# tenpy/cyten

Hardware: AMD Instinct MI355X
Metric: block-sparse tdot+SVD GFLOP/s (fp64) (higher is better)
Workload: dtype f64

## Files before the change

cyten_amd/csrc/blocked_qr.hip:

```cpp
#include "blocked_qr.h"
#include "qr_strip_chunks.h"

#include <algorithm>
#include <cstdlib>
#include <utility>

namespace cyb {
namespace {

#define GLOBAL_AS __attribute__((address_space(1)))
typedef GLOBAL_AS double* gp;
typedef const GLOBAL_AS double* gcp;
typedef double d4 __attribute__((ext_vector_type(4)));

constexpr int PNT = 512;
constexpr int PNW = PNT / 64;

__device__ __forceinline__ double wave_sum(double v)
{
#pragma unroll
    for (int o = 32; o > 0; o >>= 1) v += __shfl_xor(v, o);
    return v;
}

struct PanelDesc {
    double* Ac;
    double* V;
    double* T;
    double* tau;
    int64_t ld;
    int32_t m, j0, pw, pad;
    double* ctl = nullptr;
    const double* parts = nullptr;
    double rel2 = 0.0;
    int32_t n_parts = 0, step = 0;
};
constexpr int PANEL_V_ZEROED = 1;
constexpr int PANEL_REFLECT_ALWAYS = 2;

__global__ void __launch_bounds__(PNT) qr_panel_kernel(const PanelDesc* __restrict__ descs)
{
    __shared__ double red[PNW];
    __shared__ double s_tau, s_scale;
    __shared__ double Ts[NBK][NBK + 1];
    __shared__ double z[NBK];
    __shared__ double taus[NBK];
    const PanelDesc d = descs[blockIdx.x];
    const int tid = threadIdx.x, lane = tid & 63, wave = tid >> 6;
    gp Ac = (gp)d.Ac;
    gp V = (gp)d.V;
    const int64_t ld = d.ld;
    const int m = d.m, j0 = d.j0, pw = d.pw;
    for (int e = tid; e < NBK * (NBK + 1); e += PNT) (&Ts[0][0])[e] = 0.0;

    for (int jj = 0; jj < pw; ++jj) {
        const int col = j0 + jj;
        gp x = Ac + (int64_t)col * ld + col;
        const int L = m - col;
        double mx = 0.0;
        for (int i = 1 + tid; i < L; i += PNT) mx = fmax(mx, fabs(x[i]));
#pragma unroll
        for (int o = 32; o > 0; o >>= 1) mx = fmax(mx, __shfl_xor(mx, o));
        if (lane == 0) red[wave] = mx;
        __syncthreads();
        mx = 0.0;
#pragma unroll
        for (int q = 0; q < PNW; ++q) mx = fmax(mx, red[q]);
        __syncthreads();
        double ss = 0.0;
        if (mx > 1e-290) {
            const double inv = 1.0 / mx;
            for (int i = 1 + tid; i < L; i += PNT) {
                const double t = x[i] * inv;
                ss += t * t;
            }
        }
        ss = wave_sum(ss);
        if (lane == 0) red[wave] = ss;
        __syncthreads();
        if (tid == 0) {
            double tot = 0.0;
            for (int q = 0; q < PNW; ++q) tot += red[q];
            const double xnorm = mx * sqrt(tot);
            const double alpha = x[0];
            double t = 0.0, scale = 0.0, beta = alpha;
            if (xnorm != 0.0) {
                beta = -copysign(hypot(alpha, xnorm), alpha);
                t = (beta - alpha) / beta;
                scale = 1.0 / (alpha - beta);
            } else if ((d.pad & PANEL_REFLECT_ALWAYS) && alpha != 0.0) {
                beta = -alpha;
                t = 2.0;
            }
            s_tau = t;
            s_scale = scale;
            taus[jj] = t;
            ((gp)d.tau)[col] = t;
            x[0] = beta;
        }
        __syncthreads();
        const double tj = s_tau, scale = s_scale;
        gp v = V + (int64_t)col * ld;
        for (int i = tid; i < m; i += PNT) {
            double val = 0.0;
            if (i == col) val = 1.0;
            else if (i > col) val = (tj != 0.0) ? x[i - col] * scale : 0.0;
            v[i] = val;
        }
        __syncthreads();
        if (tj != 0.0) {
            for (int c = col + 1 + wave; c < j0 + pw; c += PNW) {
                gp a = Ac + (int64_t)c * ld + col;
                gcp vv = v + col;
                double dot = 0.0;
                for (int i = lane; i < L; i += 64) dot += vv[i] * a[i];
                dot = wave_sum(dot) * tj;
                for (int i = lane; i < L; i += 64) a[i] -= dot * vv[i];
            }
        }
        for (int i = wave; i < jj; i += PNW) {
            gcp vi = V + (int64_t)(j0 + i) * ld;
            double dot = 0.0;
            for (int r = col + lane; r < m; r += 64) dot += vi[r] * v[r];
            dot = wave_sum(dot);
            if (lane == 0) z[i] = dot;
        }
        __syncthreads();
        if (tid < jj) {
            double acc = 0.0;
            for (int l = tid; l < jj; ++l) acc += Ts[tid][l] * z[l];
            Ts[tid][jj] = -tj * acc;
        }
        if (tid == 0) Ts[jj][jj] = tj;
        __syncthreads();
    }
    for (int e = tid; e < NBK * NBK; e += PNT) ((gp)d.T)[e] = Ts[e / NBK][e % NBK];
}

#ifndef CYB_QR_READLANE
#define CYB_QR_READLANE 1
#endif
constexpr int RP_NT = 512;
constexpr int RP_RPT = 3;
constexpr int RP_NW = RP_NT / 64;

__device__ __forceinline__ double dshfl_xor(double v, int m) { return __shfl_xor(v, m); }

#ifndef CYB_QR_REDUCE_DPP
#define CYB_QR_REDUCE_DPP 1
#endif
#if CYB_QR_REDUCE_DPP
__device__ __forceinline__ void dswap32(double& a, double& b)
{
    const auto lo = __builtin_amdgcn_permlane32_swap((unsigned)__double2loint(a), (unsigned)__double2loint(b), false, false);
    const auto hi = __builtin_amdgcn_permlane32_swap((unsigned)__double2hiint(a), (unsigned)__double2hiint(b), false, false);
    a = __hiloint2double((int)hi[0], (int)lo[0]);
    b = __hiloint2double((int)hi[1], (int)lo[1]);
}
__device__ __forceinline__ void dswap16(double& a, double& b)
{
    const auto lo = __builtin_amdgcn_permlane16_swap((unsigned)__double2loint(a), (unsigned)__double2loint(b), false, false);
    const auto hi = __builtin_amdgcn_permlane16_swap((unsigned)__double2hiint(a), (unsigned)__double2hiint(b), false, false);
    a = __hiloint2double((int)hi[0], (int)lo[0]);
    b = __hiloint2double((int)hi[1], (int)lo[1]);
}
template <int CTRL, int BANKS>
__device__ __forceinline__ double ddpp(double old, double src)
{
    const int lo = __builtin_amdgcn_update_dpp(__double2loint(old), __double2loint(src), CTRL, 0xf, BANKS, false);
    const int hi = __builtin_amdgcn_update_dpp(__double2hiint(old), __double2hiint(src), CTRL, 0xf, BANKS, false);
    return __hiloint2double(hi, lo);
}
__device__ __forceinline__ double reduce_scatter16(double (&v)[16], int )
{
    double a[8];
#pragma unroll
    for (int i = 0; i < 8; ++i) {
        double x = v[i], y = v[i + 8];
        dswap32(x, y);
        a[i] = x + y;
    }
    double b[4];
#pragma unroll
    for (int i = 0; i < 4; ++i) {
        double x = a[i], y = a[i + 4];
        dswap16(x, y);
        b[i] = x + y;
    }
    constexpr int ROW_MIRROR = 0x140, ROW_HALF_MIRROR = 0x141;
    double c[2];
#pragma unroll
    for (int i = 0; i < 2; ++i) {
        const double p = ddpp<ROW_MIRROR, 0xc>(b[i], b[i + 2]);
        const double q = ddpp<ROW_MIRROR, 0x3>(b[i + 2], b[i]);
        c[i] = p + q;
    }
    const double p = ddpp<ROW_HALF_MIRROR, 0xa>(c[0], c[1]);
    const double q = ddpp<ROW_HALF_MIRROR, 0x5>(c[1], c[0]);
    double d = p + q;
    d += ddpp<0x4e, 0xf>(d, d);
    d += ddpp<0xb1, 0xf>(d, d);
    return d;
}
#else
__device__ __forceinline__ double reduce_scatter16(double (&v)[16], int lane)
{
    double a[8];
    {
        const bool hi = (lane & 32) != 0;
#pragma unroll
        for (int i = 0; i < 8; ++i) {
            const double send = hi ? v[i] : v[i + 8];
            const double keep = hi ? v[i + 8] : v[i];
            a[i] = keep + dshfl_xor(send, 32);
        }
    }
    double b[4];
    {
        const bool hi = (lane & 16) != 0;
#pragma unroll
        for (int i = 0; i < 4; ++i) {
            const double send = hi ? a[i] : a[i + 4];
            const double keep = hi ? a[i + 4] : a[i];
            b[i] = keep + dshfl_xor(send, 16);
        }
    }
    double c[2];
    {
        const bool hi = (lane & 8) != 0;
#pragma unroll
        for (int i = 0; i < 2; ++i) {
            const double send = hi ? b[i] : b[i + 2];
            const double keep = hi ? b[i + 2] : b[i];
            c[i] = keep + dshfl_xor(send, 8);
        }
    }
    double d;
    {
        const bool hi = (lane & 4) != 0;
        const double send = hi ? c[0] : c[1];
        const double keep = hi ? c[1] : c[0];
        d = keep + dshfl_xor(send, 4);
    }
    d += dshfl_xor(d, 2);
    d += dshfl_xor(d, 1);
    return d;
}
#endif

struct PanelShared {
    double wred[2][RP_NW][NBK];
    double wsum[2][NBK];
    double rowb[2][NBK];
    double Zs[NBK][NBK + 1];
    double taus[NBK];
    double Ts[NBK][NBK + 1];
};

template <int JJ, int RPT, int NT>
__device__ __forceinline__ void panel_step(double (&P)[RPT][NBK], PanelShared& sh, const PanelDesc& d, int tid)
{
    if (JJ >= d.pw) return;
    const int lane = tid & 63, wave = tid >> 6;
    const int j0 = d.j0;
    const int prow = j0 + JJ;
    constexpr int pb = JJ & 1;
#pragma unroll
    for (int h = 0; h < 2; ++h) {
        double part[16];
#pragma unroll
        for (int c = 0; c < 16; ++c) part[c] = 0.0;
#pragma unroll
        for (int q = 0; q < RPT; ++q) {
            const double x = (q == 0 && tid <= JJ) ? 0.0 : P[q][JJ];
#pragma unroll
            for (int c = 0; c < 16; ++c) part[c] += x * P[q][h * 16 + c];
        }
        const double r = reduce_scatter16(part, lane);
        if ((lane & 3) == 0) {
            const int idx = ((lane >> 5) & 1) * 8 + ((lane >> 4) & 1) * 4 + ((lane >> 3) & 1) * 2 + ((lane >> 2) & 1);
            sh.wred[pb][wave][h * 16 + idx] = r;
        }
    }
    if (tid == JJ) {
#pragma unroll
        for (int c = 0; c < NBK; ++c) sh.rowb[pb][c] = P[0][c];
    }
    __syncthreads();
#if CYB_QR_READLANE
    const int lc = lane & (NBK - 1);
    double ws = 0.0;
#pragma unroll
    for (int w = 0; w < NT / 64; ++w) ws += sh.wred[pb][w][lc];
    const double rb = sh.rowb[pb][lc];
    const double alpha = __hiloint2double(__builtin_amdgcn_readlane(__double2hiint(rb), JJ), __builtin_amdgcn_readlane(__double2loint(rb), JJ));
    const double xn2_raw = __hiloint2double(__builtin_amdgcn_readlane(__double2hiint(ws), JJ), __builtin_amdgcn_readlane(__double2loint(ws), JJ));
#else
    if (tid < NBK) {
        double t = 0.0;
#pragma unroll
        for (int w = 0; w < NT / 64; ++w) t += sh.wred[pb][w][tid];
        sh.wsum[pb][tid] = t;
    }
    __syncthreads();
    const double alpha = sh.rowb[pb][JJ];
    const double xn2_raw = sh.wsum[pb][JJ];
#endif
    const double xn2 = fma(alpha * alpha, (d.pad & PANEL_REFLECT_ALWAYS) ? 1e-40 : 0.0, xn2_raw);
    double tau = 0.0, scale = 0.0, beta = alpha;
    if (xn2 > 1e-290) {
        beta = -copysign(sqrt(alpha * alpha + xn2), alpha);
        tau = (beta - alpha) / beta;
        scale = 1.0 / (alpha - beta);
    }
    double v[RPT];
#pragma unroll
    for (int q = 0; q < RPT; ++q) {
        const double x = P[q][JJ];
        if (q == 0) {
            const bool below = tid > JJ;
            const bool pivot = tid == JJ;
            v[q] = below ? x * scale : (pivot ? 1.0 : 0.0);
            P[q][JJ] = below ? v[q] : (pivot ? beta : x);
        } else {
            v[q] = x * scale;
            P[q][JJ] = v[q];
        }
    }
#if CYB_QR_READLANE
    const double tl = tau * (rb + scale * ws);
    const int tlo = __double2loint(tl), thi = __double2hiint(tl);
#pragma unroll
    for (int c = JJ + 1; c < NBK; ++c) {
        const double t = __hiloint2double(__builtin_amdgcn_readlane(thi, c), __builtin_amdgcn_readlane(tlo, c));
#pragma unroll
        for (int q = 0; q < RPT; ++q) P[q][c] -= t * v[q];
    }
#else
#pragma unroll
    for (int c = JJ + 1; c < NBK; ++c) {
        if (c < d.pw) {
            const double t = tau * (sh.rowb[pb][c] + scale * sh.wsum[pb][c]);
#pragma unroll
            for (int q = 0; q < RPT; ++q) P[q][c] -= t * v[q];
        }
    }
#endif
#if CYB_QR_READLANE
    if (tid < JJ) sh.Zs[tid][JJ] = rb + scale * ws;
#else
    if (tid < JJ) sh.Zs[tid][JJ] = sh.rowb[pb][tid] + scale * sh.wsum[pb][tid];
#endif
    if (tid == 0) {
        sh.taus[JJ] = tau;
        ((gp)d.tau)[prow] = tau;
    }
}

template <int RPT, int NT, int... Is>
__device__ __forceinline__ void panel_steps(double (&P)[RPT][NBK], PanelShared& sh, const PanelDesc& d, int tid,
                                            std::integer_sequence<int, Is...>)
{
    (panel_step<Is, RPT, NT>(P, sh, d, tid), ...);
}

template <int RPT, int NT = RP_NT>
__device__ __forceinline__ void panel_reg_body(const PanelDesc& d, PanelShared& sh, const int tid)
{
    gp Ac = (gp)d.Ac;
    gp V = (gp)d.V;
    const int64_t ld = d.ld;
    const int m = d.m, j0 = d.j0, pw = d.pw;
    double P[RPT][NBK];
#pragma unroll
    for (int q = 0; q < RPT; ++q) {
        const int row = j0 + tid + NT * q;
        const bool ok = row < m;
        gcp src = (gcp)Ac + (int64_t)j0 * ld + (ok ? row : j0);
#pragma unroll
        for (int c = 0; c < NBK; ++c) P[q][c] = src[(int64_t)(c < pw ? c : pw - 1) * ld];
#pragma unroll
        for (int c = 0; c < NBK; ++c) {
            asm volatile("" : "+v"(P[q][c]));
            P[q][c] = (ok && c < pw) ? P[q][c] : 0.0;
        }
    }
    for (int e = tid; e < NBK * (NBK + 1); e += NT) (&sh.Zs[0][0])[e] = 0.0;
    __syncthreads();

    panel_steps<RPT, NT>(P, sh, d, tid, std::make_integer_sequence<int, NBK>{});
#pragma unroll
    for (int q = 0; q < RPT; ++q) {
        const int row = j0 + tid + NT * q;
        if (row < m) {
            gp pa = Ac + (int64_t)j0 * ld + row;
            gp pv = V + (int64_t)j0 * ld + row;
#pragma unroll
            for (int c = 0; c < NBK; ++c)
                if (c < pw) {
                    pa[(int64_t)c * ld] = P[q][c];
                    pv[(int64_t)c * ld] = (q > 0 || tid > c) ? P[q][c] : (tid == c ? 1.0 : 0.0);
                }
        }
    }
    for (int64_t e = tid; e < ((d.pad & PANEL_V_ZEROED) ? 0 : (int64_t)j0 * pw); e += NT) {
        const int c = (int)(e / j0), row = (int)(e % j0);
        V[(int64_t)(j0 + c) * ld + row] = 0.0;
    }
    __syncthreads();
    if (tid < NBK) {
        double trow[NBK];
#pragma unroll
        for (int j = 0; j < NBK; ++j) {
            double acc = 0.0;
#pragma unroll
            for (int l = 0; l < j; ++l) acc += trow[l] * sh.Zs[l][j];
            const double tj = j < pw ? sh.taus[j] : 0.0;
            trow[j] = (tid < j) ? -tj * acc : (tid == j ? tj : 0.0);
            sh.Ts[tid][j] = trow[j];
        }
    }
    __syncthreads();

    for (int e = tid; e < NBK * NBK; e += NT) ((gp)d.T)[e] = sh.Ts[e / NBK][e % NBK];
}

template <int NT, typename Desc>
__device__ __forceinline__ bool panel_stop_check(const Desc& d, double* red, int tid, bool writer = true)
{
    if (!d.ctl) return false;
    gp ctl = (gp)d.ctl;
    const double stopped = ctl[0];
    if (stopped != 0.0) return (double)d.step >= stopped - 1.0;
    if (d.n_parts <= 0) return false;
    gcp parts = (gcp)d.parts;
    double t = 0.0;
    for (int i = tid; i < d.n_parts; i += NT) t += parts[i];
#pragma unroll
    for (int o = 32; o > 0; o >>= 1) t += __shfl_xor(t, o);
    if ((tid & 63) == 0) red[tid >> 6] = t;
    __syncthreads();
    double sum = 0.0;
#pragma unroll
    for (int w = 0; w < NT / 64; ++w) sum += red[w];
    const double ref = fmax(ctl[1], sum);
    const bool stop = sum <= d.rel2 * ref;
    __syncthreads();
    if (tid == 0 && writer) {
        if (stop) ctl[0] = (double)d.step + 1.0;
        else ctl[1] = ref;
    }
    return stop;
}

__global__ void __launch_bounds__(RP_NT) qr_panel_reg_kernel(const PanelDesc* __restrict__ descs)
{
    __shared__ PanelShared sh;
    const PanelDesc d = descs[blockIdx.x];
    if (panel_stop_check<RP_NT>(d, &sh.wsum[0][0], (int)threadIdx.x)) return;
    panel_reg_body<RP_RPT>(d, sh, (int)threadIdx.x);
}
struct PanelDescM {
    double* Ac;
    double* V;
    double* T;
    double* tau;
    double* xchg;
    unsigned int* ticket;
    unsigned int* err;
    int64_t ld;
    int32_t m, j0, pw, vzero;
    int32_t wg, n_wg, pad0, pad1;
    double* ctl = nullptr;
    const double* parts = nullptr;
    double rel2 = 0.0;
    int32_t n_parts = 0, step = 0;
};
constexpr int RPM_ROWS = RP_NT * RP_RPT;

template <int JJ>
__device__ __forceinline__ void panel_step_multi(double (&P)[RP_RPT][NBK], PanelShared& sh, const PanelDescM& d, int tid)
{
    if (JJ >= d.pw) return;
    const int lane = tid & 63, wave = tid >> 6;
    const int j0 = d.j0, rbase = d.j0 + d.wg * RPM_ROWS;
    const int prow = j0 + JJ;
    constexpr int pb = JJ & 1;
#pragma unroll
    for (int h = 0; h < 2; ++h) {
        double part[16];
#pragma unroll
        for (int c = 0; c < 16; ++c) part[c] = 0.0;
#pragma unroll
        for (int q = 0; q < RP_RPT; ++q) {
            const int row = rbase + tid + RP_NT * q;
            const double x = (row <= prow) ? 0.0 : P[q][JJ];
#pragma unroll
            for (int c = 0; c < 16; ++c) part[c] += x * P[q][h * 16 + c];
        }
        const double r = reduce_scatter16(part, lane);
        if ((lane & 3) == 0) {
            const int idx = ((lane >> 5) & 1) * 8 + ((lane >> 4) & 1) * 4 + ((lane >> 3) & 1) * 2 + ((lane >> 2) & 1);
            sh.wred[pb][wave][h * 16 + idx] = r;
        }
    }
#pragma unroll
    for (int q = 0; q < RP_RPT; ++q)
        if (rbase + tid + RP_NT * q == prow) {
#pragma unroll
            for (int c = 0; c < NBK; ++c) sh.rowb[pb][c] = P[q][c];
        }
    __syncthreads();
    if (tid < NBK) {
        double t = 0.0;
#pragma unroll
        for (int w = 0; w < RP_NW; ++w) t += sh.wred[pb][w][tid];
        double* slot = d.xchg + ((size_t)JJ * d.n_wg + d.wg) * 64;
        __hip_atomic_store(slot + tid, t, __ATOMIC_RELAXED, __HIP_MEMORY_SCOPE_AGENT);
        if (d.wg == 0) __hip_atomic_store(slot + 32 + tid, sh.rowb[pb][tid], __ATOMIC_RELAXED, __HIP_MEMORY_SCOPE_AGENT);
        asm volatile("s_waitcnt vmcnt(0)" ::: "memory");
        if (tid == 0) {
            __hip_atomic_fetch_add(d.ticket + JJ, 1u, __ATOMIC_RELAXED, __HIP_MEMORY_SCOPE_AGENT);
            const unsigned long long t0 = wall_clock64();
            while (__hip_atomic_load(d.ticket + JJ, __ATOMIC_RELAXED, __HIP_MEMORY_SCOPE_AGENT) < (unsigned int)d.n_wg) {
                if (wall_clock64() - t0 > 100000000ull || __hip_atomic_load(d.err, __ATOMIC_RELAXED, __HIP_MEMORY_SCOPE_AGENT)) {
                    __hip_atomic_store(d.err, 1u, __ATOMIC_RELAXED, __HIP_MEMORY_SCOPE_AGENT);
                    break;
                }
            }
        }
        asm volatile("" ::: "memory");
        __builtin_amdgcn_wave_barrier();
        double tot = 0.0;
        for (int w = 0; w < d.n_wg; ++w)
            tot += __hip_atomic_load(d.xchg + ((size_t)JJ * d.n_wg + w) * 64 + tid, __ATOMIC_RELAXED, __HIP_MEMORY_SCOPE_AGENT);
        sh.wsum[pb][tid] = tot;
        sh.rowb[pb][tid] = __hip_atomic_load(d.xchg + (size_t)JJ * d.n_wg * 64 + 32 + tid, __ATOMIC_RELAXED, __HIP_MEMORY_SCOPE_AGENT);
    }
    __syncthreads();
    const double alpha = sh.rowb[pb][JJ];
    const double xn2 = fma(alpha * alpha, (d.vzero & PANEL_REFLECT_ALWAYS) ? 1e-40 : 0.0, sh.wsum[pb][JJ]);
    double tau = 0.0, scale = 0.0, beta = alpha;
    if (xn2 > 1e-290) {
        beta = -copysign(sqrt(alpha * alpha + xn2), alpha);
        tau = (beta - alpha) / beta;
        scale = 1.0 / (alpha - beta);
    }
    double v[RP_RPT];
#pragma unroll
    for (int q = 0; q < RP_RPT; ++q) {
        const int row = rbase + tid + RP_NT * q;
        const double x = P[q][JJ];
        const bool below = row > prow;
        const bool pivot = row == prow;
        v[q] = below ? x * scale : (pivot ? 1.0 : 0.0);
        P[q][JJ] = below ? v[q] : (pivot ? beta : x);
    }
#pragma unroll
    for (int c = JJ + 1; c < NBK; ++c) {
        if (c < d.pw) {
            const double t = tau * (sh.rowb[pb][c] + scale * sh.wsum[pb][c]);
#pragma unroll
            for (int q = 0; q < RP_RPT; ++q) P[q][c] -= t * v[q];
        }
    }
    if (tid < JJ) sh.Zs[tid][JJ] = sh.rowb[pb][tid] + scale * sh.wsum[pb][tid];
    if (tid == 0) {
        sh.taus[JJ] = tau;
        if (d.wg == 0) ((gp)d.tau)[prow] = tau;
    }
}

template <int... Is>
__device__ __forceinline__ void panel_steps_multi(double (&P)[RP_RPT][NBK], PanelShared& sh, const PanelDescM& d, int tid,
                                                  std::integer_sequence<int, Is...>)
{
    (panel_step_multi<Is>(P, sh, d, tid), ...);
}

__global__ void __launch_bounds__(RP_NT) qr_panel_multi_kernel(const PanelDescM* __restrict__ descs)
{
    __shared__ PanelShared sh;
    const PanelDescM d = descs[blockIdx.x];
    const int tid = threadIdx.x;
    if (panel_stop_check<RP_NT>(d, &sh.wsum[0][0], tid, d.wg == 0)) return;
    gp Ac = (gp)d.Ac;
    gp V = (gp)d.V;
    const int64_t ld = d.ld;
    const int m = d.m, j0 = d.j0, pw = d.pw, rbase = d.j0 + d.wg * RPM_ROWS;
    double P[RP_RPT][NBK];
#pragma unroll
    for (int q = 0; q < RP_RPT; ++q) {
        const int row = rbase + tid + RP_NT * q;
#pragma unroll
        for (int c = 0; c < NBK; ++c) P[q][c] = (row < m && c < pw) ? Ac[(int64_t)(j0 + c) * ld + row] : 0.0;
    }
    for (int e = tid; e < NBK * (NBK + 1); e += RP_NT) (&sh.Zs[0][0])[e] = 0.0;
    __syncthreads();
    panel_steps_multi(P, sh, d, tid, std::make_integer_sequence<int, NBK>{});
#pragma unroll
    for (int q = 0; q < RP_RPT; ++q) {
        const int row = rbase + tid + RP_NT * q;
        if (row < m) {
#pragma unroll
            for (int c = 0; c < NBK; ++c)
                if (c < pw) {
                    const int col = j0 + c;
                    Ac[(int64_t)col * ld + row] = P[q][c];
                    V[(int64_t)col * ld + row] = (row > col) ? P[q][c] : (row == col ? 1.0 : 0.0);
                }
        }
    }
    if (d.wg == 0 && !(d.vzero & PANEL_V_ZEROED))
        for (int64_t e = tid; e < (int64_t)j0 * pw; e += RP_NT) {
            const int c = (int)(e / j0), row = (int)(e % j0);
            V[(int64_t)(j0 + c) * ld + row] = 0.0;
        }
    __syncthreads();
    if (tid < NBK) {
        double trow[NBK];
#pragma unroll
        for (int j = 0; j < NBK; ++j) {
            double acc = 0.0;
#pragma unroll
            for (int l = 0; l < j; ++l) acc += trow[l] * sh.Zs[l][j];
            const double tj = j < pw ? sh.taus[j] : 0.0;
            trow[j] = (tid < j) ? -tj * acc : (tid == j ? tj : 0.0);
            sh.Ts[tid][j] = trow[j];
        }
    }
    __syncthreads();
    if (d.wg == 0)
        for (int e = tid; e < NBK * NBK; e += RP_NT) ((gp)d.T)[e] = sh.Ts[e / NBK][e % NBK];
}

constexpr int RP_WAVE_RPT = 3;
constexpr int RP_WAVE_ROWS = 64 * RP_WAVE_RPT;
__global__ void __launch_bounds__(64) qr_panel_wave_kernel(const PanelDesc* __restrict__ descs)
{
    __shared__ PanelShared sh;
    const PanelDesc d = descs[blockIdx.x];
    if (panel_stop_check<64>(d, &sh.wsum[0][0], (int)threadIdx.x)) return;
    panel_reg_body<RP_WAVE_RPT, 64>(d, sh, (int)threadIdx.x);
}
__global__ void __launch_bounds__(128) qr_panel_wave2_kernel(const PanelDesc* __restrict__ descs)
{
    __shared__ PanelShared sh;
    const PanelDesc d = descs[blockIdx.x];
    if (panel_stop_check<128>(d, &sh.wsum[0][0], (int)threadIdx.x)) return;
    panel_reg_body<RP_WAVE_RPT, 128>(d, sh, (int)threadIdx.x);
}
__global__ void __launch_bounds__(256) qr_panel_wave4_kernel(const PanelDesc* __restrict__ descs)
{
    __shared__ PanelShared sh;
    const PanelDesc d = descs[blockIdx.x];
    if (panel_stop_check<256>(d, &sh.wsum[0][0], (int)threadIdx.x)) return;
    panel_reg_body<RP_WAVE_RPT, 256>(d, sh, (int)threadIdx.x);
}

struct StripDesc {
    double* C;
    const double* V;
    const double* T;
    int64_t ldc, ldv;
    int32_t mr, nc, pw, transT;
    const double* ctl = nullptr;
    double* part_out = nullptr;
    int32_t step = 0, pad2 = 0;
};
constexpr int ST_NT = 512;
constexpr int ST_NW = ST_NT / 64;
constexpr int ST_LS = NBK + 1;
constexpr int ST_UN = 4;

template <bool NORM>
__global__ void __launch_bounds__(ST_NT) reflector_strip_kernel(const StripDesc* __restrict__ descs)
{
    __shared__ double part[ST_NW][NBK][ST_LS];
    __shared__ double W1s[NBK][ST_LS], W2s[NBK][ST_LS], Ps[NBK][ST_LS];
    const StripDesc d = descs[blockIdx.x];
    if (d.ctl) {
        const double stopped = *(gcp)d.ctl;
        if (stopped != 0.0 && (double)d.step >= stopped - 1.0) return;
    }
    const int tid = threadIdx.x, lane = tid & 63, wave = tid >> 6;
    const int x = lane & 15, kq = lane >> 4;
    gcp V = (gcp)d.V;
    gp C = (gp)d.C;
    gcp T = (gcp)d.T;
    const int mr = d.mr, nc = d.nc, pw = d.pw;
    const int64_t ldv = d.ldv, ldc = d.ldc;
    for (int e = tid; e < NBK * NBK; e += ST_NT) {
        const int a = e / NBK, b = e % NBK;
        Ps[a][b] = T[d.transT ? b * NBK + a : e];
    }
    {
        const int64_t vo0 = (int64_t)(x < pw ? x : 0) * ldv, vo1 = (int64_t)(x + 16 < pw ? x + 16 : 0) * ldv;
        const int64_t co0 = (int64_t)(x < nc ? x : 0) * ldc, co1 = (int64_t)(x + 16 < nc ? x + 16 : 0) * ldc;
        d4 acc[2][2];
#pragma unroll
        for (int i = 0; i < 2; ++i)
#pragma unroll
            for (int j = 0; j < 2; ++j) acc[i][j] = d4{0.0, 0.0, 0.0, 0.0};
        const int nstep = (mr + 7) / 8;
        double va[ST_UN][2][2], ca[ST_UN][2][2], vn[ST_UN][2][2], cn[ST_UN][2][2];
        auto load = [&](double (&v)[ST_UN][2][2], double (&c)[ST_UN][2][2], int s0) {
#pragma unroll
            for (int u = 0; u < ST_UN; ++u) {
                const int i = (s0 + ST_NW * u) * 8 + 2 * kq;
#pragma unroll
                for (int h = 0; h < 2; ++h) {
                    const bool ok = i + h < mr;
                    const int ii = ok ? i + h : 0;
                    v[u][0][h] = ok ? V[vo0 + ii] : 0.0;
                    v[u][1][h] = ok ? V[vo1 + ii] : 0.0;
                    c[u][0][h] = ok ? C[co0 + ii] : 0.0;
                    c[u][1][h] = ok ? C[co1 + ii] : 0.0;
                }
            }
        };
        if (wave < nstep) load(va, ca, wave);
        for (int s0 = wave; s0 < nstep; s0 += ST_NW * ST_UN) {
            const bool more = s0 + ST_NW * ST_UN < nstep;
            if (more) load(vn, cn, s0 + ST_NW * ST_UN);
#pragma unroll
            for (int u = 0; u < ST_UN; ++u) {
                if (s0 + ST_NW * u < nstep) {
#pragma unroll
                    for (int h = 0; h < 2; ++h)
#pragma unroll
                        for (int i = 0; i < 2; ++i)
#pragma unroll
                            for (int j = 0; j < 2; ++j)
                                acc[i][j] = __builtin_amdgcn_mfma_f64_16x16x4f64(va[u][i][h], ca[u][j][h], acc[i][j], 0, 0, 0);
                }
            }
            if (more) {
#pragma unroll
                for (int u = 0; u < ST_UN; ++u)
#pragma unroll
                    for (int i = 0; i < 2; ++i)
#pragma unroll
                        for (int h = 0; h < 2; ++h) {
                            va[u][i][h] = vn[u][i][h];
                            ca[u][i][h] = cn[u][i][h];
                        }
            }
        }
#pragma unroll
        for (int i = 0; i < 2; ++i)
#pragma unroll
            for (int j = 0; j < 2; ++j)
#pragma unroll
                for (int r = 0; r < 4; ++r) part[wave][i * 16 + kq + 4 * r][j * 16 + x] = acc[i][j][r];
    }
    __syncthreads();
    for (int e = tid; e < NBK * NBK; e += ST_NT) {
        const int a = e / NBK, c = e % NBK;
        double t = 0.0;
#pragma unroll
        for (int w = 0; w < ST_NW; ++w) t += part[w][a][c];
        W1s[a][c] = t;
    }
    __syncthreads();
    if (wave < 4) {
        const int ta = wave >> 1, tc = wave & 1;
        d4 acc = d4{0.0, 0.0, 0.0, 0.0};
#pragma unroll
        for (int kk = 0; kk < NBK / 4; ++kk)
            acc = __builtin_amdgcn_mfma_f64_16x16x4f64(Ps[ta * 16 + x][4 * kk + kq], W1s[4 * kk + kq][tc * 16 + x], acc, 0, 0, 0);
#pragma unroll
        for (int r = 0; r < 4; ++r) W2s[ta * 16 + kq + 4 * r][tc * 16 + x] = acc[r];
    }
    __syncthreads();
    {
        double w2[2][NBK / 4];
#pragma unroll
        for (int ct = 0; ct < 2; ++ct)
#pragma unroll
            for (int kk = 0; kk < NBK / 4; ++kk) w2[ct][kk] = -W2s[4 * kk + kq][ct * 16 + x];
        int64_t vcol[NBK / 4], ccol[2][4];
#pragma unroll
        for (int kk = 0; kk < NBK / 4; ++kk) vcol[kk] = (int64_t)(4 * kk + kq < pw ? 4 * kk + kq : 0) * ldv;
#pragma unroll
        for (int ct = 0; ct < 2; ++ct)
#pragma unroll
            for (int r = 0; r < 4; ++r) {
                const int c = ct * 16 + kq + 4 * r;
                ccol[ct][r] = (int64_t)(c < nc ? c : 0) * ldc;
            }
        const int ntile = (mr + 15) / 16;
        struct Tile {
            double v[NBK / 4];
            d4 c[2];
        };
        auto load = [&](Tile& t, int rt) {
            const int i = rt * 16 + x;
            const bool ok = i < mr;
            const int ii = ok ? i : 0;
#pragma unroll
            for (int kk = 0; kk < NBK / 4; ++kk) t.v[kk] = ok ? V[vcol[kk] + ii] : 0.0;
#pragma unroll
            for (int ct = 0; ct < 2; ++ct)
#pragma unroll
                for (int r = 0; r < 4; ++r) t.c[ct][r] = C[ccol[ct][r] + ii];
        };
        double nrm2 = 0.0;
        auto finish = [&](Tile& t, int rt) {
#pragma unroll
            for (int kk = 0; kk < NBK / 4; ++kk) {
                t.c[0] = __builtin_amdgcn_mfma_f64_16x16x4f64(w2[0][kk], t.v[kk], t.c[0], 0, 0, 0);
                t.c[1] = __builtin_amdgcn_mfma_f64_16x16x4f64(w2[1][kk], t.v[kk], t.c[1], 0, 0, 0);
            }
            const int i = rt * 16 + x;
            if (i < mr) {
                const double below = i >= pw ? 1.0 : 0.0;
#pragma unroll
                for (int ct = 0; ct < 2; ++ct)
#pragma unroll
                    for (int r = 0; r < 4; ++r)
                        if (ct * 16 + kq + 4 * r < nc) {
                            C[ccol[ct][r] + i] = t.c[ct][r];
                            if constexpr (NORM) nrm2 = fma(below * t.c[ct][r], t.c[ct][r], nrm2);
                        }
            }
        };
        Tile t0, t1, t2;
        if (wave < ntile) load(t0, wave);
        if (wave + ST_NW < ntile) load(t1, wave + ST_NW);
        for (int rt = wave; rt < ntile; rt += 3 * ST_NW) {
            if (rt + 2 * ST_NW < ntile) load(t2, rt + 2 * ST_NW);
            finish(t0, rt);
            if (rt + ST_NW < ntile) {
                if (rt + 3 * ST_NW < ntile) load(t0, rt + 3 * ST_NW);
                finish(t1, rt + ST_NW);
            }
            if (rt + 2 * ST_NW < ntile) {
                if (rt + 4 * ST_NW < ntile) load(t1, rt + 4 * ST_NW);
                finish(t2, rt + 2 * ST_NW);
            }
        }
        if constexpr (NORM) if (d.part_out) {
#pragma unroll
            for (int o = 32; o > 0; o >>= 1) nrm2 += __shfl_xor(nrm2, o);
            __syncthreads();
            if (lane == 0) W1s[0][wave] = nrm2;
            __syncthreads();
            if (tid == 0) {
                double t = 0.0;
#pragma unroll
                for (int w = 0; w < ST_NW; ++w) t += W1s[0][w];
                *(gp)d.part_out = t;
            }
        }
    }
}

struct ChunkDesc {
    double* C;
    const double* V;
    const double* T;
    double* wpart;
    int64_t ldc, ldv;
    int32_t mr, nc, pw, transT;
    int32_t slot, n_slots, row0, step;
    const double* ctl;
    double* part_out;
};

__global__ void __launch_bounds__(ST_NT) strip_w1_kernel(const ChunkDesc* __restrict__ descs)
{
    __shared__ double part[ST_NW][NBK][ST_LS];
    const ChunkDesc d = descs[blockIdx.x];
    if (d.ctl) {
        const double stopped = *(gcp)d.ctl;
        if (stopped != 0.0 && (double)d.step >= stopped - 1.0) return;
    }
    const int tid = threadIdx.x, lane = tid & 63, wave = tid >> 6;
    const int x = lane & 15, kq = lane >> 4;
    gcp V = (gcp)d.V;
    gp C = (gp)d.C;
    const int mr = d.mr, nc = d.nc, pw = d.pw;
    const int64_t ldv = d.ldv, ldc = d.ldc;
    {
        const int64_t vo0 = (int64_t)(x < pw ? x : 0) * ldv, vo1 = (int64_t)(x + 16 < pw ? x + 16 : 0) * ldv;
        const int64_t co0 = (int64_t)(x < nc ? x : 0) * ldc, co1 = (int64_t)(x + 16 < nc ? x + 16 : 0) * ldc;
        d4 acc[2][2];
#pragma unroll
        for (int i = 0; i < 2; ++i)
#pragma unroll
            for (int j = 0; j < 2; ++j) acc[i][j] = d4{0.0, 0.0, 0.0, 0.0};
        const int nstep = (mr + 7) / 8;
        double va[ST_UN][2][2], ca[ST_UN][2][2], vn[ST_UN][2][2], cn[ST_UN][2][2];
        auto load = [&](double (&v)[ST_UN][2][2], double (&c)[ST_UN][2][2], int s0) {
#pragma unroll
            for (int u = 0; u < ST_UN; ++u) {
                const int i = (s0 + ST_NW * u) * 8 + 2 * kq;
#pragma unroll
                for (int h = 0; h < 2; ++h) {
                    const bool ok = i + h < mr;
                    const int ii = ok ? i + h : 0;
                    v[u][0][h] = ok ? V[vo0 + ii] : 0.0;
                    v[u][1][h] = ok ? V[vo1 + ii] : 0.0;
                    c[u][0][h] = ok ? C[co0 + ii] : 0.0;
                    c[u][1][h] = ok ? C[co1 + ii] : 0.0;
                }
            }
        };
        if (wave < nstep) load(va, ca, wave);
        for (int s0 = wave; s0 < nstep; s0 += ST_NW * ST_UN) {
            const bool more = s0 + ST_NW * ST_UN < nstep;
            if (more) load(vn, cn, s0 + ST_NW * ST_UN);
#pragma unroll
            for (int u = 0; u < ST_UN; ++u) {
                if (s0 + ST_NW * u < nstep) {
#pragma unroll
                    for (int h = 0; h < 2; ++h)
#pragma unroll
                        for (int i = 0; i < 2; ++i)
#pragma unroll
                            for (int j = 0; j < 2; ++j)
                                acc[i][j] = __builtin_amdgcn_mfma_f64_16x16x4f64(va[u][i][h], ca[u][j][h], acc[i][j], 0, 0, 0);
                }
            }
            if (more) {
#pragma unroll
                for (int u = 0; u < ST_UN; ++u)
#pragma unroll
                    for (int i = 0; i < 2; ++i)
#pragma unroll
                        for (int h = 0; h < 2; ++h) {
                            va[u][i][h] = vn[u][i][h];
                            ca[u][i][h] = cn[u][i][h];
                        }
            }
        }
#pragma unroll
        for (int i = 0; i < 2; ++i)
#pragma unroll
            for (int j = 0; j < 2; ++j)
#pragma unroll
                for (int r = 0; r < 4; ++r) part[wave][i * 16 + kq + 4 * r][j * 16 + x] = acc[i][j][r];
    }
    __syncthreads();
    gp out = (gp)d.wpart + (size_t)d.slot * (NBK * NBK);
    for (int e = tid; e < NBK * NBK; e += ST_NT) {
        const int a = e / NBK, c = e % NBK;
        double t = 0.0;
#pragma unroll
        for (int w = 0; w < ST_NW; ++w) t += part[w][a][c];
        out[e] = t;
    }
}

template <bool NORM>
__global__ void __launch_bounds__(ST_NT) strip_apply_kernel(const ChunkDesc* __restrict__ descs)
{
    __shared__ double W1s[NBK][ST_LS], W2s[NBK][ST_LS], Ps[NBK][ST_LS];
    const ChunkDesc d = descs[blockIdx.x];
    if (d.ctl) {
// ... 833 lines not shown
```

Measured before the change: 6144.

## Compute panel Gram upper-right block with MFMA instead of per-step reductions

For panel steps at index 16 and beyond, the per-step dot-product reduction now covers only the second half of the columns. The V-times-V cross block needed for the T factor (Zs columns 16..31) is instead computed after the panel with f64 MFMA on V rows staged through LDS, interleaved with the V/Ac writeback. This is meant to remove half the scalar FMA and shuffle-reduction work in the later panel steps. In exchange it adds LDS staging, wave barriers and extra shared memory per block, which may reduce occupancy.

```diff
diff --git a/cyten_amd/csrc/blocked_qr.hip b/cyten_amd/csrc/blocked_qr.hip
--- a/cyten_amd/csrc/blocked_qr.hip
+++ b/cyten_amd/csrc/blocked_qr.hip
@@ -265,8 +265,9 @@
     const int j0 = d.j0;
     const int prow = j0 + JJ;
     constexpr int pb = JJ & 1;
-#pragma unroll
-    for (int h = 0; h < 2; ++h) {
+    constexpr int H0 = JJ >= 16 ? 1 : 0;
+#pragma unroll
+    for (int h = H0; h < 2; ++h) {
         double part[16];
 #pragma unroll
         for (int c = 0; c < 16; ++c) part[c] = 0.0;
@@ -288,7 +289,7 @@
     }
     __syncthreads();
 #if CYB_QR_READLANE
-    const int lc = lane & (NBK - 1);
+    const int lc = (lane & (NBK - 1)) | (H0 * 16);
     double ws = 0.0;
 #pragma unroll
     for (int w = 0; w < NT / 64; ++w) ws += sh.wred[pb][w][lc];
@@ -296,7 +297,7 @@
     const double alpha = __hiloint2double(__builtin_amdgcn_readlane(__double2hiint(rb), JJ), __builtin_amdgcn_readlane(__double2loint(rb), JJ));
     const double xn2_raw = __hiloint2double(__builtin_amdgcn_readlane(__double2hiint(ws), JJ), __builtin_amdgcn_readlane(__double2loint(ws), JJ));
 #else
-    if (tid < NBK) {
+    if (tid >= H0 * 16 && tid < NBK) {
         double t = 0.0;
 #pragma unroll
         for (int w = 0; w < NT / 64; ++w) t += sh.wred[pb][w][tid];
@@ -347,9 +348,9 @@
     }
 #endif
 #if CYB_QR_READLANE
-    if (tid < JJ) sh.Zs[tid][JJ] = rb + scale * ws;
+    if (tid >= H0 * 16 && tid < JJ) sh.Zs[tid][JJ] = rb + scale * ws;
 #else
-    if (tid < JJ) sh.Zs[tid][JJ] = sh.rowb[pb][tid] + scale * sh.wsum[pb][tid];
+    if (tid >= H0 * 16 && tid < JJ) sh.Zs[tid][JJ] = sh.rowb[pb][tid] + scale * sh.wsum[pb][tid];
 #endif
     if (tid == 0) {
         sh.taus[JJ] = tau;
@@ -364,8 +365,65 @@
     (panel_step<Is, RPT, NT>(P, sh, d, tid), ...);
 }
 
+constexpr int GS_LD = NBK + 2;
+template <int NT>
+struct PanelGramStage {
+    double t[NT / 64][16 * GS_LD];
+};
+
+struct PanelGramLane {
+    double* wr;
+    const double* rd;
+    int grp;
+};
+template <int NT>
+__device__ __forceinline__ PanelGramLane panel_gram_lane(PanelGramStage<NT>& gs, int tid)
+{
+    const int lane = tid & 63, wave = __builtin_amdgcn_readfirstlane(tid >> 6);
+    const int grp = lane >> 4, col = lane & 15;
+    double* st = gs.t[wave];
+    return PanelGramLane{st + col * GS_LD, st + (8 * (grp & 1) + 4 * (grp >> 1)) * GS_LD + col, grp};
+}
+__device__ __forceinline__ void panel_gram_chunk(const double (&Pq)[NBK], const PanelGramLane& g, int t, d4& acc)
+{
+    if (g.grp == t) {
+#pragma unroll
+        for (int c = 0; c < NBK; c += 2) {
+            double2 w2;
+            w2.x = Pq[c];
+            w2.y = Pq[c + 1];
+            *reinterpret_cast<double2*>(g.wr + c) = w2;
+        }
+    }
+    __builtin_amdgcn_wave_barrier();
+#pragma unroll
+    for (int s = 0; s < 4; ++s) {
+        const double a = g.rd[s * GS_LD], b = g.rd[s * GS_LD + 16];
+        acc = __builtin_amdgcn_mfma_f64_16x16x4f64(a, b, acc, 0, 0, 0);
+    }
+    __builtin_amdgcn_wave_barrier();
+}
+template <int NT>
+__device__ __forceinline__ void panel_gram_publish(PanelGramStage<NT>& gs, const d4& acc, int tid)
+{
+    const int lane = tid & 63, wave = __builtin_amdgcn_readfirstlane(tid >> 6);
+#pragma unroll
+    for (int i = 0; i < 4; ++i) gs.t[wave][((lane >> 4) + 4 * i) * 16 + (lane & 15)] = acc[i];
+}
+
+template <int NT>
+__device__ __forceinline__ void panel_gram_sum(const PanelGramStage<NT>& gs, PanelShared& sh, int tid)
+{
+    for (int e = tid; e < 256; e += NT) {
+        double t = 0.0;
+#pragma unroll
+        for (int w = 0; w < NT / 64; ++w) t += gs.t[w][e];
+        sh.Zs[e >> 4][16 + (e & 15)] = t;
+    }
+}
+
 template <int RPT, int NT = RP_NT>
-__device__ __forceinline__ void panel_reg_body(const PanelDesc& d, PanelShared& sh, const int tid)
+__device__ __forceinline__ void panel_reg_body(const PanelDesc& d, PanelShared& sh, PanelGramStage<NT>& gs, const int tid)
 {
     gp Ac = (gp)d.Ac;
     gp V = (gp)d.V;
@@ -389,25 +447,48 @@
     __syncthreads();
 
     panel_steps<RPT, NT>(P, sh, d, tid, std::make_integer_sequence<int, NBK>{});
+    const bool gram = pw > 16;
+    const PanelGramLane gl = panel_gram_lane<NT>(gs, tid);
+    const int wrow = j0 + 64 * __builtin_amdgcn_readfirstlane(tid >> 6);
+    d4 acc = {0.0, 0.0, 0.0, 0.0};
 #pragma unroll
     for (int q = 0; q < RPT; ++q) {
         const int row = j0 + tid + NT * q;
-        if (row < m) {
-            gp pa = Ac + (int64_t)j0 * ld + row;
-            gp pv = V + (int64_t)j0 * ld + row;
-#pragma unroll
-            for (int c = 0; c < NBK; ++c)
-                if (c < pw) {
-                    pa[(int64_t)c * ld] = P[q][c];
-                    pv[(int64_t)c * ld] = (q > 0 || tid > c) ? P[q][c] : (tid == c ? 1.0 : 0.0);
-                }
-        }
-    }
+        const bool ok = row < m;
+        gp pa = Ac + (int64_t)j0 * ld + row;
+        gp pv = V + (int64_t)j0 * ld + row;
+        if (q == 0) {
+            if (ok) {
+#pragma unroll
+                for (int c = 0; c < NBK; ++c)
+                    if (c < pw) pa[(int64_t)c * ld] = P[q][c];
+            }
+#pragma unroll
+            for (int c = 0; c < NBK; ++c) P[q][c] = tid > c ? P[q][c] : (tid == c && c < pw ? 1.0 : 0.0);
+        }
+#pragma unroll
+        for (int t = 0; t < 4; ++t) {
+            if (gram && wrow + NT * q + 16 * t < m) panel_gram_chunk(P[q], gl, t, acc);
+            if (ok) {
+#pragma unroll
+                for (int c = 8 * t; c < 8 * t + 8; ++c)
+                    if (c < pw) {
+                        if (q > 0) pa[(int64_t)c * ld] = P[q][c];
+                        pv[(int64_t)c * ld] = P[q][c];
+                    }
+            }
+        }
+    }
+    if (gram) panel_gram_publish<NT>(gs, acc, tid);
     for (int64_t e = tid; e < ((d.pad & PANEL_V_ZEROED) ? 0 : (int64_t)j0 * pw); e += NT) {
         const int c = (int)(e / j0), row = (int)(e % j0);
         V[(int64_t)(j0 + c) * ld + row] = 0.0;
     }
     __syncthreads();
+    if (gram) {
+        panel_gram_sum<NT>(gs, sh, tid);
+        __syncthreads();
+    }
     if (tid < NBK) {
         double trow[NBK];
 #pragma unroll
@@ -456,9 +537,10 @@
 __global__ void __launch_bounds__(RP_NT) qr_panel_reg_kernel(const PanelDesc* __restrict__ descs)
 {
     __shared__ PanelShared sh;
+    __shared__ PanelGramStage<RP_NT> gs;
     const PanelDesc d = descs[blockIdx.x];
     if (panel_stop_check<RP_NT>(d, &sh.wsum[0][0], (int)threadIdx.x)) return;
-    panel_reg_body<RP_RPT>(d, sh, (int)threadIdx.x);
+    panel_reg_body<RP_RPT>(d, sh, gs, (int)threadIdx.x);
 }
 struct PanelDescM {
     double* Ac;
@@ -639,23 +721,26 @@
 __global__ void __launch_bounds__(64) qr_panel_wave_kernel(const PanelDesc* __restrict__ descs)
 {
     __shared__ PanelShared sh;
+    __shared__ PanelGramStage<64> gs;
     const PanelDesc d = descs[blockIdx.x];
     if (panel_stop_check<64>(d, &sh.wsum[0][0], (int)threadIdx.x)) return;
-    panel_reg_body<RP_WAVE_RPT, 64>(d, sh, (int)threadIdx.x);
+    panel_reg_body<RP_WAVE_RPT, 64>(d, sh, gs, (int)threadIdx.x);
 }
 __global__ void __launch_bounds__(128) qr_panel_wave2_kernel(const PanelDesc* __restrict__ descs)
 {
     __shared__ PanelShared sh;
+    __shared__ PanelGramStage<128> gs;
     const PanelDesc d = descs[blockIdx.x];
     if (panel_stop_check<128>(d, &sh.wsum[0][0], (int)threadIdx.x)) return;
-    panel_reg_body<RP_WAVE_RPT, 128>(d, sh, (int)threadIdx.x);
+    panel_reg_body<RP_WAVE_RPT, 128>(d, sh, gs, (int)threadIdx.x);
 }
 __global__ void __launch_bounds__(256) qr_panel_wave4_kernel(const PanelDesc* __restrict__ descs)
 {
     __shared__ PanelShared sh;
+    __shared__ PanelGramStage<256> gs;
     const PanelDesc d = descs[blockIdx.x];
     if (panel_stop_check<256>(d, &sh.wsum[0][0], (int)threadIdx.x)) return;
-    panel_reg_body<RP_WAVE_RPT, 256>(d, sh, (int)threadIdx.x);
+    panel_reg_body<RP_WAVE_RPT, 256>(d, sh, gs, (int)threadIdx.x);
 }
 
 struct StripDesc {
```

After: 6204 (median of 6 runs). About the same (+1.0%).
